# microsoft/aurora

Measured on AMD Instinct MI355X. Metric: forecast-steps/sec (6h step) 0.25deg ERA5 721x1440x13, higher is better.
Workload: dtype bf16; 1 GPU; AuroraPretrained(autocast=True) 1.3B, 0.25deg ERA5 721x1440, 13 levels, T=2, batch 1 per GPU, one forward step (BASELINE.json configs[1]); parallelism=1 GPU

## Files before the change

aurora_amd/csrc/model.h:

```cpp
#pragma once

#include <math.h>
#include <stdlib.h>
#include <string.h>

#include <algorithm>
#include <array>
#include <exception>
#include <map>
#include <memory>
#include <stdexcept>
#include <string>
#include <vector>

#include "band.h"
#include "common.h"

namespace aurora {

struct Fail {
  int code;
};
#define REQUIRE(cond, ...)               \
  do {                                   \
// ... 73 lines not shown
struct Resampler {
  struct Layer {
    const float *to_q, *to_kv, *to_out, *fc1_w, *fc1_b, *fc2_w, *fc2_b, *ln1_w, *ln1_b, *ln2_w, *ln2_b;
    const float *ln_k_w = nullptr, *ln_k_b = nullptr, *ln_q_w = nullptr, *ln_q_b = nullptr;
    int inner, head_dim, hidden, dim, ctx_dim;
    float v_l1;
    int f16_mode;
    const void *to_kv_s = nullptr, *to_out_s = nullptr, *fc1_s = nullptr, *fc2_s = nullptr;
  };
  std::vector<Layer> layers;
  std::vector<DevBuf> own;
  DevBuf vs_w, vs_ws;
  int n_s = 0, n_vs = 0, vs_lq = 0;
};

enum SrcKind { SRC_SURF, SRC_STATIC, SRC_DYN, SRC_ATMOS };
struct Channel {
  std::string name;
  SrcKind kind;
  int src;
  int transform;
  float tw0 = 0.f, tw1 = 0.f, tb = 0.f;
};
struct EmbedPack {
  DevBuf w, ws;
  int K = 0, Kpad = 0, groups = 1;
  float l1 = 0.f;
  std::vector<int> channels;
};
struct HeadGroup {
  std::vector<std::string> names;
  DevBuf w, b;
  int groups = 1;
  DevBuf ws, bs;
  int n_pad = 0;
};

struct DevTables { DevBuf tok, grp; int n_windows = 0, n_tok = 0; bool has_grp = false; };
struct DevPlan {
  DevBuf tok, grp, send_idx;
  int n_windows = 0, n_tok = 0, n_own = 0, n_halo = 0, n_interior = 0;
  int recv_off[2] = {0, 0}, recv_cnt[2] = {0, 0}, send_cnt[2] = {0, 0};
  bool has_grp = false;
};

}

struct aurora_hip_model {
  int D = 0, P = 0, Cl = 0, perceiver_heads = 0, n_stages = 0;
  int enc_depths[4] = {0}, dec_depths[4] = {0}, enc_heads[4] = {0}, dec_heads[4] = {0}, window[3] = {0};
  int enc_depth = 1, dec_depth = 1, max_history = 2, lora_steps = 40, lora_mode = 0;
// ... 35 lines not shown
  std::vector<double> static_loc;
  std::map<std::array<int64_t, 3>, aurora::EmbedPack> embed_packs;
  float enc_bias_max = 0.f;
  aurora::DevBuf surf_w0_s, surf_w2_s;
  float surf_l1_0 = 0.f, surf_b0 = 0.f, surf_c = 0.f;
  bool surf_chain = false;
  aurora::HeadGroup head_surf, head_main, head_alt;
  float dec_out_bound = 0.f, dec_out_bound_alt = 0.f;
  std::map<std::pair<int, int>, aurora::DevTables> tables;
  std::vector<aurora::Res> stage_res;
  std::vector<std::array<int, 2>> merge_pad;

  aurora_hip_band band{0, 1, nullptr, nullptr, nullptr};
  std::vector<std::vector<std::array<int, 2>>> rows;
  std::map<std::pair<int, int>, aurora::DevPlan> plans;
  void* stage_send = nullptr;
  void* stage_recv = nullptr;
  int64_t staging_bytes = 0, staging_need = 0;
  bool sharded() const { return band.world > 1; }
  int fuse_ln = 1;
  bool split_attention = false;
  bool qkv_planes = true;
  bool reassoc_out = true;
  bool score_weights = true;

  aurora::DevBuf abs_enc, dyn_planes, ctx_max;
  aurora::DevBuf tickets;
  bool split_k = true;
  int abs_B = 0;
  struct Pinned { float* host = nullptr; size_t bytes = 0; hipEvent_t done = nullptr; };
  Pinned pinned[4];
  int pinned_next = 0;
  ~aurora_hip_model() {
    for (auto& t : timed) { (void)hipEventDestroy(t.e0); (void)hipEventDestroy(t.e1); }
    for (auto& e : event_pool) (void)hipEventDestroy(e);
    for (auto& s : pinned) {
      if (s.host) (void)hipHostFree(s.host);
      if (s.done) (void)hipEventDestroy(s.done);
    }
  }
  aurora::Arena arena;
  bool dry = false;
  int64_t generation = 0;

  struct Timed { int kind; double work; hipEvent_t e0, e1; };
  uint32_t profile_mask = 0;
// ... 121 lines not shown
  std::vector<float> h(n);
  hip_ok(hipMemcpy(h.data(), dev, n * 4, hipMemcpyDeviceToHost), "download");
  return h;
}
inline std::vector<float> to_host(const Tensor& t) { return to_host(t.f(), (size_t)t.numel); }
inline bool contains(const std::vector<std::string>& v, const std::string& s) { return std::find(v.begin(), v.end(), s) != v.end(); }

constexpr float F16_SAFE = 16384.0f;
constexpr float PRESPLIT_W_MAX = 1000.0f;
int bounded_mode();
std::string level_to_str(double level);

int lora_key(const Model& m, int step);
float absmax(const float* dev, size_t n);
float absmax(const std::vector<float>& h);
inline float absmax(const Tensor& t) { return absmax(t.f(), (size_t)t.numel); }
float max_row_l1(const std::vector<float>& h, int64_t rows, int64_t K, float floor);
bool presplit_shape(int64_t rows, int64_t K, int row_multiple);
DevBuf presplit(const float* w, int64_t rows, int64_t K, int64_t ld, int row_multiple, int groups = 1);
void score_weights(Model& m, Resampler& r, const float* q0, int Lq, int heads);
void build_atmos_heads(Model& m, bool per_level);
const AttnSet& attn_weights(Model& m, int key, void* stream);
const EmbedPack& embed_pack(Model& m, int kind, int T, const std::vector<char>& present);
enum Expansion { POS, SCALE, LEAD_TIME, LEVELS, ABS_TIME };
void fourier(Expansion kind, const double* x, int64_t n, int d, float* out);
const DevTables& tables_for(Model& m, int stage, bool shifted);
const DevPlan& plan_for(Model& m, int stage, bool shifted);
struct StepIO {
  const aurora_hip_step_io* io;
  int B, T;
};
void run_step(Model& m, const StepIO& s, void* stream);

}
```

aurora_amd/csrc/model.hip:

```cpp
#include "model.h"

namespace aurora {

hipEvent_t take_event(Model& m) {
  if (!m.event_pool.empty()) {
    hipEvent_t e = m.event_pool.back();
    m.event_pool.pop_back();
    return e;
  }
  hipEvent_t e;
  hip_ok(hipEventCreate(&e), "hipEventCreate");
  return e;
}

int bounded_mode() {
  static const int mode = getenv("AURORA_F32_GEMM") ? -1 : 2;
  return mode;
}

std::string level_to_str(double level) {
  const double value = round(level * 1000.0) / 1000.0;
  char buf[64];
  if (value == (double)(long long)value) snprintf(buf, sizeof buf, "%lld", (long long)value);
  else {
// ... 153 lines not shown
    names(c->density_channel_surf_vars, c->n_density, m->density_vars);
    names(c->angle_surf_vars, c->n_angle, m->angle_vars);
    if (m->surf_inputs.empty()) m->surf_inputs = m->surf_vars;
    REQUIRE(m->variant == 2 || m->surf_inputs == m->surf_vars, "create: surf_inputs are for the ocean-wave variant");
    if (c->difference_history)
      for (int i = 0; i < c->n_modulation_heads; ++i)
        if (c->difference_history[i] >= 0) m->diff_index[m->mod_heads[i]] = c->difference_history[i];
    REQUIRE(m->static_vars.size() <= 60 && m->surf_inputs.size() <= 60 && m->atmos_vars.size() <= 60, "create: too many variables");
    build_blocks(*m);
    build_channels(*m);
    m->ctx_max = DevBuf(16);
    const auto& tu = c->tuning;
    REQUIRE(tu.fuse_ln >= 0 && tu.fuse_ln <= 3, "create: tuning.fuse_ln = %d (0 default, 1 never, 2 by the fill rule, 3 always)", tu.fuse_ln);
    auto sw = [](int32_t v, bool dflt, const char* what) {
      REQUIRE(v >= 0 && v <= 2, "create: tuning.%s = %d (0 default, 1 off, 2 on)", what, v);
      return v == 0 ? dflt : v == 2;
    };
    m->fuse_ln = tu.fuse_ln == 0 ? 1 : tu.fuse_ln - 1;
    m->split_attention = sw(tu.band_split_attention, false, "band_split_attention");
    m->qkv_planes = sw(tu.qkv_planes, true, "qkv_planes");
    m->split_k = sw(tu.split_k, true, "split_k");
    m->reassoc_out = sw(tu.perceiver_reassoc, true, "perceiver_reassoc");
    m->score_weights = sw(tu.score_weights, true, "score_weights");
    m->tickets = DevBuf(SPLIT_TICKETS * sizeof(int32_t));
    hip_ok(hipMemset(m->tickets.p, 0, SPLIT_TICKETS * sizeof(int32_t)), "hipMemset");
    *out = m.release();
  })
}

extern "C" void aurora_hip_destroy(aurora_hip_model* m) { delete m; }

extern "C" int aurora_hip_set_band(aurora_hip_model* mp, const aurora_hip_band* band) {
  GUARDED({
    REQUIRE(mp != nullptr, "set_band: null model");
    Model& m = *mp;
    if (band == nullptr || band->world <= 1) {
      m.band = aurora_hip_band{0, 1, nullptr, nullptr, nullptr};
    } else {
      REQUIRE(band->rank >= 0 && band->rank < band->world, "set_band: rank %d of %d", band->rank, band->world);
      REQUIRE(band->post && band->wait, "set_band: the halo transport callbacks are required");
      m.band = *band;
    }
    m.have_grid = false;
    m.plans.clear(); m.rows.clear();
    m.stage_send = m.stage_recv = nullptr;
    m.staging_bytes = m.staging_need = 0;
// ... 150 lines not shown
```

aurora_amd/csrc/model_weights.hip:

```cpp
#include "model.h"

namespace aurora {

constexpr int LORA_RANK = 8;

float absmax(const std::vector<float>& h) {
  float mx = 0.f;
  for (float v : h) mx = std::max(mx, fabsf(v));
  return mx;
}
float absmax(const float* dev, size_t n) { return absmax(to_host(dev, n)); }
float max_row_l1(const std::vector<float>& h, int64_t rows, int64_t K, float floor) {
  float best = floor;
  for (int64_t r = 0; r < rows; ++r) {
    float sum = 0.f;
    for (int64_t k = 0; k < K; ++k) sum += fabsf(h[(size_t)r * K + k]);
    best = std::max(best, sum);
  }
  return best;
}

bool presplit_shape(int64_t rows, int64_t K, int row_multiple) { return rows % row_multiple == 0 && K % 32 == 0 && K >= 96; }
DevBuf presplit(const float* w, int64_t rows, int64_t K, int64_t ld, int row_multiple, int groups) {
  if (!presplit_shape(rows, K, row_multiple)) return DevBuf();
// ... 173 lines not shown
        hip_ok(hipStreamSynchronize(as_stream(stream)), "sync");
        src = merged.f();
      }
      const void* use = src;
      if (m.autocast) {
        DevBuf h((size_t)out_f * in_f * 2);
        ok(aurora_hip_convert(src, h.p, out_f * in_f, AURORA_F32, stream));
        hip_ok(hipStreamSynchronize(as_stream(stream)), "sync");
        use = h.p;
        set.own.push_back(std::move(h));
      } else if (key >= 0) {
        set.own.push_back(std::move(merged));
      }
      (which == 0 ? set.qkv : set.proj).push_back(use);
    }
  }
  while (m.attn_sets.size() > 3) {
    bool erased = false;
    for (auto jt = m.attn_sets.begin(); jt != m.attn_sets.end(); ++jt)
      if (jt->first != -1) { m.attn_sets.erase(jt); erased = true; break; }
    if (!erased) break;
  }
  return m.attn_sets.emplace(key, std::move(set)).first->second;
}

const EmbedPack& embed_pack(Model& m, int kind, int T, const std::vector<char>& present) {
  const std::vector<Channel>& chans = kind == 0 ? m.surf_channels : m.atmos_channels;
  int64_t mask = 0, mask_hi = 0;
  REQUIRE(chans.size() <= 126, "more than 126 input channels");
  for (size_t i = 0; i < chans.size(); ++i)
    if (present[i]) (i < 63 ? mask : mask_hi) |= (int64_t)1 << (i % 63);
  const std::array<int64_t, 3> key{(int64_t)kind * 1024 + T, mask, mask_hi};
  auto it = m.embed_packs.find(key);
  if (it != m.embed_packs.end()) return it->second;
  EmbedPack pk;
  for (size_t i = 0; i < chans.size(); ++i)
    if (present[i]) pk.channels.push_back((int)i);
  REQUIRE(!pk.channels.empty(), "no %s variable given", kind == 0 ? "surface-level" : "atmospheric");
  const bool per_level = kind == 1 && !m.level_condition.empty();
  pk.groups = per_level ? m.n_levels : 1;
  const int V = (int)pk.channels.size(), PP = m.P * m.P;
  pk.K = V * T * PP;
  pk.Kpad = round_up(pk.K, 32);
  std::vector<float> host((size_t)pk.groups * m.D * pk.Kpad, 0.f);
  for (int g = 0; g < pk.groups; ++g) {
    const std::string prefix = kind == 0 ? "encoder.surf_token_embeds.weights."
                               : per_level ? "encoder.atmos_token_embeds.layers." + level_to_str(m.levels[g]) + ".weights."
                                           : "encoder.atmos_token_embeds.weights.";
    for (int v = 0; v < V; ++v) {
      const Tensor& t = m.T_(prefix + chans[pk.channels[v]].name);
      REQUIRE(t.shape.size() == 5 && t.shape[0] == m.D && t.shape[2] >= T && t.shape[3] == m.P, "bad patch-embed weight shape");
      const int64_t Tmax = t.shape[2];
      const std::vector<float> wv = to_host(t);
      for (int d = 0; d < m.D; ++d)
        for (int tt = 0; tt < T; ++tt)
          memcpy(&host[((size_t)g * m.D + d) * pk.Kpad + ((size_t)v * T + tt) * PP], &wv[((size_t)d * Tmax + tt) * PP], PP * sizeof(float));
    }
  }
  pk.l1 = max_row_l1(host, (int64_t)pk.groups * m.D, pk.Kpad, 1e-6f);
  pk.w = to_device(host);
  if (bounded_mode() == 2 && absmax(host) < PRESPLIT_W_MAX)
    pk.ws = presplit(pk.w.f(), m.D, pk.Kpad, pk.Kpad, 256, pk.groups);
  return m.embed_packs.emplace(key, std::move(pk)).first->second;
}

void build_atmos_heads(Model& m, bool per_level) {
  std::vector<std::string> sep = m.sep_perceiver, main_names, alt_names;
  if (!m.mod_heads.empty())
    for (const auto& v : m.sep_perceiver) sep.push_back(v + "_mod");
  for (const auto& n : m.atmos_heads) (contains(sep, n) ? alt_names : main_names).push_back(n);
  build_heads(m, m.head_main, "atmos", main_names, per_level);
  build_heads(m, m.head_alt, "atmos", alt_names, per_level);
}

namespace {

void surface_mlp_chain(Model& m) {
  const Tensor &t0 = m.T_("encoder.surf_mlp.net.0.weight"), &t2 = m.T_("encoder.surf_mlp.net.2.weight");
  const std::vector<float> w0 = to_host(t0), w2 = to_host(t2);
  const int64_t N0 = t0.shape[0], K0 = t0.shape[1];
  m.surf_l1_0 = max_row_l1(w0, N0, K0, 1e-6f);
  m.surf_b0 = absmax(m.T_("encoder.surf_mlp.net.0.bias"));
  m.surf_c = absmax(m.T_("encoder.surf_token_embeds.bias")) + absmax(m.T_("encoder.surf_level_encoding"));
  m.surf_chain = bounded_mode() == 2 && absmax(w0) < PRESPLIT_W_MAX && absmax(w2) < PRESPLIT_W_MAX &&
                 presplit_shape(N0, K0, 256) && presplit_shape(K0, N0, 256);
// ... 62 lines not shown
                1e-5f, AURORA_F32);
  hip_ok(hipStreamSynchronize(as_stream(L.stream)), "precompute sync");
  score_weights(m, m.enc_rs, m.enc_q0.f(), n_lat, m.perceiver_heads);
  m.has_alt = !m.sep_perceiver.empty();
  if (m.has_alt) m.dec_rs_alt = pack_resampler(m, "decoder.level_decoder_alternate", m.dec_depth, m.perceiver_heads);
}

void feature_combiners(Model& m) {
  for (int kind = 0; kind < 2; ++kind)
    for (Channel& ch : kind == 0 ? m.surf_channels : m.atmos_channels)
      if (ch.transform == 2) {
        const std::string p = std::string(kind == 0 ? "surf" : "atmos") + "_feature_combiner." + ch.name;
        const std::vector<float> wv = to_host(m.T_(p + ".weight")), bv = to_host(m.T_(p + ".bias"));
        REQUIRE(wv.size() == 2 && bv.size() == 1, "bad feature combiner shape for %s", p.c_str());
        ch.tw0 = wv[0]; ch.tw1 = wv[1]; ch.tb = bv[0];
      }
}

}

}

using namespace aurora;

extern "C" int aurora_hip_pack_weights(aurora_hip_model* m, const char* name, const void* data, const int64_t* shape, int ndim,
                                       int dtype, int on_device) {
  GUARDED({
    REQUIRE(m && name && data && ndim >= 0 && ndim <= 8, "pack_weights: bad argument");
    REQUIRE(dtype == AURORA_F32, "pack_weights: parameters must be float32 (the engine keeps fp32 masters)");
    Tensor t;
    t.numel = 1;
    for (int i = 0; i < ndim; ++i) { t.shape.push_back(shape[i]); t.numel *= shape[i]; }
    t.buf = DevBuf((size_t)t.numel * 4);
    hip_ok(hipMemcpy(t.buf.p, data, (size_t)t.numel * 4, on_device ? hipMemcpyDeviceToDevice : hipMemcpyHostToDevice),
           "pack_weights copy");
    m->w[name] = std::move(t);
    m->finalized = false;
  })
}

namespace {
const char PACK_MAGIC[] = "AURORAHIP1";

bool backbone_matrix(const Model& m, const std::string& name) {
  if (name.rfind("backbone.", 0) != 0 || name.size() < 7 || name.compare(name.size() - 7, 7, ".weight") != 0) return false;
  for (const char* tag : {".mlp.fc1.", ".mlp.fc2.", ".downsample.reduction.", ".upsample.lin1.", ".upsample.lin2."})
// ... 103 lines not shown
```

aurora_amd/csrc/step.hip:

```cpp
#include <algorithm>

#include "model.h"
#include "resampler_space.h"

namespace aurora {

namespace {

struct CtxGuard { const float* word; float a, c, limit_kv; bool pairs; };

LayerSpace layer_space(const Model& m, const Resampler& rs, size_t i, int B, int64_t cols, int64_t ctx_rows, int Lq, int Lk,
                       int heads) {
  const auto& ly = rs.layers[i];
  LayerShape sh{};
  sh.layer = i;
  sh.dim = ly.dim; sh.inner = ly.inner; sh.hidden = ly.hidden; sh.head_dim = ly.head_dim; sh.heads = heads;
  sh.n_vs = rs.n_vs; sh.vs_lq = rs.vs_lq;
  sh.ln_k = ly.ln_k_w != nullptr; sh.to_out_s = ly.to_out_s != nullptr; sh.fc1_s = ly.fc1_s != nullptr; sh.fc2_s = ly.fc2_s != nullptr;
  sh.f16_mode = ly.f16_mode;
  sh.reassoc_out = m.reassoc_out;
  sh.out_supported = aurora_hip_perceiver_out_supported(Lq, Lk, heads, ly.head_dim, ly.dim) != 0;
  sh.B = B; sh.cols = cols; sh.ctx_rows = ctx_rows; sh.Lq = Lq; sh.Lk = Lk;
  return layer_space(sh);
}

void resampler_mlp(Model& m, Launcher& L, const Resampler::Layer& ly, const LayerSpace& sp, const float* o, const float* res,
                   int64_t res_mod, float* lat1, char* S, float* y, int64_t n_rows, float eps, bool y_pairs) {
  const int Dd = ly.dim;
  if (sp.pairs)
    timed(m, L.stream, K_LAYERNORM, 0.0, [&] {
      return aurora_hip_layernorm_split(o, Dd, ly.ln1_w, ly.ln1_b, res, Dd, res_mod, 0, nullptr, 0, lat1, Dd, n_rows, Dd, eps, L.stream);
    });
  else L.layernorm(o, Dd, ly.ln1_w, ly.ln1_b, res, Dd, res_mod, lat1, Dd, nullptr, 0, n_rows, Dd, eps, AURORA_F32);
  float* hid = (float*)S;
  const int64_t chunk_rows = sp.chunk_rows;
  REQUIRE(chunk_rows >= 1 && (size_t)chunk_rows * sp.hid_row <= sp.s_bytes, "resampler: scratch region too small for the MLP");
  const int all = 2 | AURORA_F32_A_SPLIT | AURORA_F32_W_SPLIT;
  for (int64_t r0 = 0; r0 < n_rows; r0 += chunk_rows) {
    const int64_t nr = std::min(chunk_rows, n_rows - r0);
    LinearOp fc1(lat1 + (size_t)r0 * Dd, Dd, sp.pairs ? ly.fc1_s : ly.fc1_w, Dd, ly.fc1_b, hid, ly.hidden, nr, ly.hidden, Dd, AURORA_F32);
    LinearOp fc2(hid, ly.hidden, sp.pairs ? ly.fc2_s : ly.fc2_w, ly.hidden, ly.fc2_b, y + (size_t)r0 * Dd, Dd, nr, Dd, ly.hidden, AURORA_F32);
    L.linear(fc1.activation(AURORA_ACT_GELU).f32_mode(sp.pairs ? all | AURORA_F32_C_SPLIT : ly.f16_mode));
    L.linear(fc2.f32_mode(sp.pairs ? all : ly.f16_mode));
  }
  if (sp.pairs)
    timed(m, L.stream, K_LAYERNORM, 0.0, [&] {
      return aurora_hip_layernorm_split(y, Dd, ly.ln2_w, ly.ln2_b, lat1, Dd, 0, 1, y_pairs ? nullptr : y, Dd, y_pairs ? y : nullptr, Dd,
                                        n_rows, Dd, eps, L.stream);
    });
  else L.layernorm(y, Dd, ly.ln2_w, ly.ln2_b, lat1, Dd, 0, y, Dd, nullptr, 0, n_rows, Dd, eps, AURORA_F32);
}

float* resampler(Model& m, Launcher& L, const Resampler& rs, const float* ctx, int64_t ctx_rows, int ctx_dim, const float* q0,
                 const float* latents0, int B, int64_t cols, int64_t kv_bstride, int64_t kv_lstride, int Lq, int Lk, int heads,
                 float eps, const CtxGuard* cg = nullptr, bool out_pairs = false, int own_word = 0, bool scan_ctx = true) {
  const int64_t n_cols = (int64_t)B * cols, n_rows = n_cols * Lq;
  const float* ctx_max = cg ? cg->word : m.ctx_max.f() + own_word;
  const float g_a = cg ? cg->a : 1.0f, g_c = cg ? cg->c : 0.0f;
  const bool ctx_pairs = cg && cg->pairs;
  if (!cg && scan_ctx)
    timed(m, L.stream, K_ABSMAX, 0.0, [&] { return aurora_hip_absmax_fold(ctx, ctx_rows * ctx_dim, m.ctx_max.f() + own_word, L.stream); });
  float* lat = nullptr;
  for (size_t i = 0; i < rs.layers.size(); ++i) {
    const auto& ly = rs.layers[i];
    const int inner = ly.inner, Dd = ly.dim;
    const LayerSpace sp = layer_space(m, rs, i, B, cols, ctx_rows, Lq, Lk, heads);
    const bool scores = sp.scores;
    const int kv_ld = sp.kv_ld;
    float* y = (float*)m.arena.take(sp.unit);
    const size_t after_y = m.arena.top;
    float* lat1 = (float*)m.arena.take(sp.unit);
    char* S = (char*)m.arena.take(sp.s_bytes);
    float* kv = (float*)S;
    auto guarded = [&](const float* A, int64_t lda, const float* Wf, const void* Ws, float* C_, int64_t ldc, int64_t M_, int N_,
                       int K_, float limit, bool a_pairs = false) {
      LinearOp op(A, lda, Wf, K_, nullptr, C_, ldc, M_, N_, K_, AURORA_F32);
      if (Ws) {
        L.guarded_pair(op, Ws, a_pairs ? AURORA_F32_A_SPLIT : 0, ctx_max, limit);
      } else if (ly.f16_mode == 2) {
        L.linear(op.f32_mode(2).guarded_by(ctx_max, limit));
      } else {
        L.linear(op.f32_mode(ly.f16_mode));
      }
    };
    REQUIRE(!ctx_pairs || ly.to_kv_s, "resampler: a pair-layout context needs pre-split to_kv weights");
    guarded(ctx, ctx_dim, scores ? rs.vs_w.f() : ly.to_kv, scores ? rs.vs_ws.p : ly.to_kv_s, kv, kv_ld, ctx_rows, kv_ld, ctx_dim,
            ctx_pairs ? cg->limit_kv : (F16_SAFE - g_c) / g_a, ctx_pairs);
    if (ly.ln_k_w)
      L.layernorm(kv, 2 * inner, ly.ln_k_w, ly.ln_k_b, nullptr, 0, 0, kv, 2 * inner, nullptr, 0, ctx_rows, inner, 1e-5f,
                  AURORA_F32);
    const float* q = q0;
    int64_t q_stride = 0;
    if (i > 0) {
      float* qb = (float*)(S + round256(sp.kv_bytes));
      L.linear(LinearOp(lat, Dd, ly.to_q, Dd, nullptr, qb, inner, n_rows, inner, Dd, AURORA_F32));
      if (ly.ln_q_w) L.layernorm(qb, inner, ly.ln_q_w, ly.ln_q_b, nullptr, 0, 0, qb, inner, nullptr, 0, n_rows, inner, 1e-5f, AURORA_F32);
      q = qb;
      q_stride = Lq;
    }
    float* att = sp.att_in_y ? y : (float*)(S + sp.att_off);
    const float lim_out = (F16_SAFE / ly.v_l1 - g_c) / g_a;
    float* o = (float*)S;
    if (sp.reassoc) {
      REQUIRE(sp.p_off >= sp.kv_bytes && sp.p_off >= sp.unit && sp.p_off + sp.p_bytes <= sp.s_bytes,
              "resampler: the softmax weights overlap k | v or to_out's result in the scratch region");
      float* P = (float*)(S + sp.p_off);
      void* Vp = y;
      timed(m, L.stream, K_PERCEIVER_ATTENTION, 0.0, [&] {
        if (scores)
          return aurora_hip_perceiver_probs_scores(kv, kv_ld, inner, P, Vp, B, cols, kv_bstride, kv_lstride, Lq, Lk, heads, ly.head_dim,
                                                   ctx_max, lim_out, L.stream);
        return aurora_hip_perceiver_probs(q, kv, P, Vp, B, cols, kv_bstride, kv_lstride, Lq, Lk, heads, ly.head_dim, ctx_max, lim_out,
                                          L.stream);
      });
      timed(m, L.stream, K_PERCEIVER_OUT, 2.0 * (double)n_cols * Lk * Dd * inner + 2.0 * (double)n_rows * Dd * heads * Lk, [&] {
        return aurora_hip_perceiver_out(Vp, ly.to_out_s, inner, P, nullptr, o, Dd, n_cols, Lq, Lk, heads, ly.head_dim, Dd, ctx_max,
                                        lim_out, L.stream);
      });
      timed(m, L.stream, K_PERCEIVER_ATTENTION, 0.0, [&] {
        if (scores)
          return aurora_hip_perceiver_attention_scores(kv, kv_ld, inner, att, B, cols, kv_bstride, kv_lstride, Lq, Lk, heads,
                                                       ly.head_dim, nullptr, 0.f, ctx_max, lim_out, L.stream);
        return aurora_hip_perceiver_attention_unless(q, q_stride, kv, att, B, cols, kv_bstride, kv_lstride, Lq, Lk, heads,
                                                     ly.head_dim, AURORA_F32, nullptr, 0.f, ctx_max, lim_out, L.stream);
// ... 130 lines not shown
    const float lim_e = F16_SAFE, lim_0 = (F16_SAFE - m.surf_c) / l1e, lim_2 = ((F16_SAFE - m.surf_b0) / m.surf_l1_0 - m.surf_c) / l1e;
    L.guarded_pair(embed, ps.ws.p, 0, word, lim_e);
    L.guarded_pair(fc1, m.surf_w0_s.p, 0, word, lim_0);
    L.guarded_pair(fc2, m.surf_w2_s.p, 0, word, lim_2);
  } else {
    L.linear(embed);
    L.linear(fc1);
    L.linear(fc2);
  }
  L.layernorm(y, D, m.W("encoder.surf_norm.weight"), m.W("encoder.surf_norm.bias"), xs0, D, 0, y, D, nullptr, 0, R, D, 1e-5f,
              AURORA_F32);
  return y;
}

const float* encode_levels(Step& s) {
  Model& m = s.m;
  Launcher& L = s.L;
  const int B = s.B, D = s.D, C = s.C;
  float* A_a;
  const EmbedPack& pa = embed_input(s, true, A_a);
  const int Kpad_a = pa.Kpad;
  bool chain = pa.ws.p != nullptr;
  for (const auto& ly : m.enc_rs.layers) chain = chain && ly.f16_mode == 2 && ly.to_kv_s != nullptr;
  float* word = m.ctx_max.f() + 1;
  patchify(s, pa, true, A_a, chain ? word : nullptr);
  float* xa = (float*)m.arena.take((size_t)C * B * s.Lp * D * 4);
  const int64_t R = (int64_t)B * s.Lp;
  CtxGuard cg{};
  const int64_t sw = pa.groups > 1 ? (int64_t)D * Kpad_a : 0;
  const LinearOp embed = LinearOp(A_a, Kpad_a, pa.w.f(), Kpad_a, m.enc_bias.f(), xa, D, R, D, Kpad_a, AURORA_F32)
                             .batched(C, R * Kpad_a, sw, D, R * D);
  if (chain) {
    const float l1 = pa.l1, cb = m.enc_bias_max;
    cg = CtxGuard{word, l1, cb, std::min(F16_SAFE, (F16_SAFE - cb) / l1), true};
    L.guarded_pair(embed, pa.ws.p, AURORA_F32_C_SPLIT, cg.word, cg.limit_kv);
  } else {
    L.linear(embed);
  }
  return resampler(m, L, m.enc_rs, xa, (int64_t)C * R, D, m.enc_q0.f(), m.W("encoder.atmos_latents"), B, s.Lp, s.Lp, R, s.Cl - 1, C,
                   m.perceiver_heads, m.ln_eps, chain ? &cg : nullptr);
}

void assemble(Step& s, const float* xs1, const float* lat, float* x_f, void* x_b) {
  Model& m = s.m;
  const int B = s.B, D = s.D;
  float* time_emb = (float*)m.arena.take((size_t)B * D * 4);
  s.L.linear(LinearOp(m.abs_enc.f(), D, m.W("encoder.absolute_time_embed.weight"), D, m.W("encoder.absolute_time_embed.bias"), time_emb,
                      D, B, D, D, AURORA_F32).residual(m.lead_emb.f(), 0));
  timed(m, s.L.stream, K_ASSEMBLE, 0.0, [&] {
    return aurora_hip_assemble_tokens(xs1, lat, m.pos_scale.f(), time_emb, x_f, x_b, B, s.Cl, s.Lp, D, s.bb, s.L.stream);
// ... 397 lines not shown
```

aurora_amd/engine/lib.py:

```python

from __future__ import annotations

import ctypes
import os
import threading
from collections import OrderedDict, namedtuple
from ctypes import c_float, c_int, c_int32, c_int64, c_void_p
from pathlib import Path
from typing import Optional

import numpy as np
import torch

F32, BF16, F64 = 0, 1, 2
ACT_NONE, ACT_GELU, ACT_SILU = 0, 1, 2

_LIB_PATH = Path(__file__).resolve().parents[1] / "_lib" / "libaurora_hip.so"


class PatchVar(ctypes.Structure):
    _fields_ = [
        ("src", c_void_p), ("stride_b", c_int64), ("stride_t", c_int64), ("stride_c", c_int64),
        ("stride_h", c_int64), ("stride_w", c_int64), ("loc", c_void_p), ("inv_scale", c_void_p),
        ("transform", c_int32), ("tw0", c_float), ("tw1", c_float), ("tb", c_float),
# ... 1320 lines not shown
    with torch.cuda.device(dev):
        order = [what for what, _ in groups if what in addr]
        table = _plane_table("diagnostics", tuple(a for what in order for a in addr[what]), dev)
        at, first = {}, table.data_ptr()
        for what in order:
            at[what], first = first, first + 8 * len(addr[what])
        moved = 4.0 * n_lat * n_lon * (n_wind * (2 + sum(k in addr for k in ("vo", "div", "ws"))) +
                                       n_cols * (C * (1 + sum(k in addr for k in ("col_u", "col_v"))) +
                                                 sum(k in addr for k in ("tcwv", "ivtu", "ivtv", "ivt"))))
        with _Timed("diagnostics", moved):
            _check(load().aurora_hip_diagnostics(at.get("u"), at.get("v"), at.get("vo"), at.get("div"), at.get("ws"), n_wind,
                                                 _ptr(row_table), float(L), 1 if wrap else 0, at.get("q"), at.get("col_u"),
                                                 at.get("col_v"), at.get("tcwv"), at.get("ivtu"), at.get("ivtv"), at.get("ivt"),
                                                 n_cols, C, _ptr(level_w), n_lat, n_lon, _stream()))


_PD =ctypes.POINTER(ctypes.c_double)
_PF = ctypes.POINTER(ctypes.c_float)
_PS = ctypes.POINTER(ctypes.c_char_p)


class HipTuning(ctypes.Structure):
    _fields_ = [("fuse_ln", c_int32), ("band_split_attention", c_int32), ("qkv_planes", c_int32), ("split_k", c_int32),
                ("perceiver_reassoc", c_int32), ("score_weights", c_int32), ("reserved", c_int32 * 2)]


def tuning_from_env() -> HipTuning:
    t = HipTuning()

    def value(var: str, allowed: tuple[int, ...]):
        raw = os.environ.get(var)
        if raw is None:
            return None
        try:
            v = int(raw.strip())
        except ValueError:
            v = None
        if v not in allowed:
            raise ValueError(f"{var}={raw!r}: expected one of {', '.join(map(str, allowed))}")
        return v

    v = value("AURORA_FUSE_LN", (0, 1, 2))
    if v is not None:
        t.fuse_ln = v + 1
    for field, var in (("band_split_attention", "AURORA_BAND_SPLIT_ATTENTION"), ("qkv_planes", "AURORA_QKV_PLANES"),
                       ("split_k", "AURORA_SPLIT_K"), ("perceiver_reassoc", "AURORA_PERCEIVER_REASSOC"),
                       ("score_weights", "AURORA_SCORE_WEIGHTS")):
        v = value(var, (0, 1))
        if v is not None:
            setattr(t, field, 2 if v else 1)
    return t


class HipConfig(ctypes.Structure):
    _fields_ = [("embed_dim", c_int32), ("patch_size", c_int32), ("latent_levels", c_int32), ("num_heads", c_int32),
                ("n_stages", c_int32), ("encoder_depths", c_int32 * 4), ("encoder_heads", c_int32 * 4),
                ("decoder_depths", c_int32 * 4), ("decoder_heads", c_int32 * 4), ("window", c_int32 * 3),
                ("enc_depth", c_int32), ("dec_depth", c_int32), ("perceiver_ln_eps", c_float),
                ("max_history", c_int32), ("timestep_hours", ctypes.c_double), ("stabilise_level_agg", c_int32),
                ("use_lora", c_int32), ("lora_steps", c_int32), ("lora_mode", c_int32), ("autocast", c_int32),
                ("n_surf", c_int32), ("n_static", c_int32), ("n_atmos", c_int32),
                ("surf_vars", _PS), ("static_vars", _PS), ("atmos_vars", _PS),
                ("variant", c_int32), ("n_level_condition", c_int32), ("level_condition", _PD),
                ("dynamic_vars", c_int32), ("atmos_static_vars", c_int32), ("clamp_at_first_step", c_int32),
                ("simulate_indexing_bug", c_int32),
                ("n_separate_perceiver", c_int32), ("separate_perceiver", _PS),
                ("n_modulation_heads", c_int32), ("modulation_heads", _PS),
                ("difference_history", ctypes.POINTER(c_int32)),
                ("n_positive_surf", c_int32), ("positive_surf_vars", _PS),
                ("n_positive_atmos", c_int32), ("positive_atmos_vars", _PS),
# ... 41 lines not shown


PROFILE_KINDS = ("linear_bf16", "linear_f32", "window_attention_bf16", "layernorm", "merge_ln", "split_ln", "patchify",
                 "perceiver_attention", "assemble_tokens", "unpatchify", "copy2d", "absmax", "linear_layernorm_bf16",
                 "gather_rows", "perceiver_out")

_SIGNATURES.update({
    "aurora_hip_profile_begin": (c_int, [c_void_p, ctypes.c_uint32]),
    "aurora_hip_profile_end": (c_int, [c_void_p, ctypes.POINTER(HipProfileEntry), c_int, ctypes.POINTER(c_int)]),
    "aurora_hip_profile_end_list": (c_int, [c_void_p, ctypes.POINTER(HipProfileEntry), c_int, ctypes.POINTER(c_int)]),
    "aurora_hip_create": (c_int, [ctypes.POINTER(HipConfig), ctypes.POINTER(c_void_p)]),
    "aurora_hip_destroy": (None, [c_void_p]),
    "aurora_hip_pack_weights": (c_int, [c_void_p, ctypes.c_char_p, c_void_p, ctypes.POINTER(c_int64), c_int, c_int, c_int]),
    "aurora_hip_finalize": (c_int, [c_void_p, c_void_p]),
    "aurora_hip_save_packed": (c_int, [c_void_p, ctypes.c_char_p, c_void_p]),
    "aurora_hip_load_packed": (c_int, [c_void_p, ctypes.c_char_p]),
    "aurora_hip_precompute": (c_int, [c_void_p, ctypes.POINTER(HipGrid), c_void_p]),
    "aurora_hip_set_time": (c_int, [c_void_p, _PD, c_int, c_void_p]),
    "aurora_hip_step": (c_int, [c_void_p, ctypes.POINTER(HipStepIO), c_void_p]),
    "aurora_hip_workspace_bytes": (c_int64, [c_void_p]),
    "aurora_hip_guard_words": (c_int, [c_void_p, ctypes.POINTER(c_float), c_void_p]),
    "aurora_hip_abi_sizes": (c_int, [ctypes.POINTER(c_int32), c_int]),
    "aurora_hip_generation": (c_int64, [c_void_p]),
    "aurora_hip_output_vars": (c_int, [c_void_p, _PS, c_int]),
    "aurora_hip_set_time_ex": (c_int, [c_void_p, _PD, ctypes.POINTER(c_int32), c_int, c_void_p]),
    "aurora_hip_set_band": (c_int, [c_void_p, ctypes.POINTER(HipBand)]),
    "aurora_hip_band_rows": (c_int, [c_void_p, ctypes.POINTER(c_int32), ctypes.POINTER(c_int32)]),
    "aurora_hip_band_staging_bytes": (c_int64, [c_void_p]),
    "aurora_hip_set_band_staging": (c_int, [c_void_p, c_void_p, c_void_p, c_int64]),
    "aurora_hip_pos_scale_encoding": (c_int, [_PD, _PD, c_int, c_int, c_int, c_int, _PF, _PF]),
    "aurora_hip_band_partition": (c_int, [c_int, ctypes.POINTER(c_int32), ctypes.POINTER(c_int32), c_int, c_int, c_int,
                                          ctypes.POINTER(c_int32), ctypes.POINTER(c_int32)]),
    "aurora_hip_band_plan": (c_int, [ctypes.POINTER(c_int32), ctypes.POINTER(c_int32), c_int, c_int, c_int,
                                     ctypes.POINTER(c_int32), ctypes.POINTER(HipPlanInfo), c_void_p, c_void_p, c_void_p,
                                     c_void_p]),
})
EXPORTED_SYMBOLS = tuple(_SIGNATURES)
```

aurora_amd/engine/native.py:

```python
from __future__ import annotations

import ctypes
from datetime import timedelta

import numpy as np
import torch

from aurora_amd import normalisation
from aurora_amd.batch import BandBatch, Batch, derive_metadata
from aurora_amd.engine import encodings, lib

_LORA_MODES = {"single": 0, "from_second": 1, "all": 2}
_VARIANTS = {"base": 0, "air_pollution": 1, "wave": 2}


def _version(t: torch.Tensor) -> int:
    try:
        return t._version
    except RuntimeError:
        return -1


def _strs(names):
    return (ctypes.c_char_p * max(len(names), 1))(*[n.encode() for n in names])
# ... 275 lines not shown
        lib._check(lib.load().aurora_hip_profile_end(self._h, out, len(out), ctypes.byref(n)))
        return {e.kernel.decode(): {"launches": e.launches, "ms": e.ms, "work": e.work} for e in out[:n.value] if e.launches}

    def profile_end_list(self) -> list:
        n = ctypes.c_int(0)
        lib._check(lib.load().aurora_hip_profile_end_list(self._h, None, 0, ctypes.byref(n)))
        out = (lib.HipProfileEntry * max(n.value, 1))()
        lib._check(lib.load().aurora_hip_profile_end_list(self._h, out, n.value, ctypes.byref(n)))
        return [(e.kernel.decode(), e.ms, e.work) for e in out[:n.value]]

    def set_time(self, times) -> None:
        stamps = _dbl([t.timestamp() / 3600 for t in times])
        cal = _i32([x for t in times for x in (t.hour, t.weekday(), t.day)])
        lib._check(lib.load().aurora_hip_set_time_ex(self._h, stamps, cal, len(times), lib._stream()))

    def workspace_bytes(self) -> int:
        return int(lib.load().aurora_hip_workspace_bytes(self._h))

    def guard_words(self) -> tuple[float, float, float, float]:
        out = (ctypes.c_float * 4)()
        lib._check(lib.load().aurora_hip_guard_words(self._h, out, lib._stream()))
        return tuple(float(v) for v in out)

    def generation(self) -> int:
        return int(lib.load().aurora_hip_generation(self._h))

    @torch.no_grad()
    def step(self, batch: Batch, upload_time: bool = True, out=None) -> Batch:
        cfg = self.cfg
        md = batch.metadata
        levels = tuple(md.atmos_levels)
        H, W = batch.spatial_shape
        first = next(iter(batch.surf_vars.values()))
        B, T = first.shape[:2]
        dev = first.device
        assert md.lat.shape[0] == H and md.lon.shape[-1] == W
        assert md.lat.dtype in (torch.float32, torch.float64), f"Latitude num. unstable: {md.lat.dtype}."
        assert md.lon.dtype in (torch.float32, torch.float64), f"Longitude num. unstable: {md.lon.dtype}."
        if self.shard is None:
            self.precompute(md.lat, md.lon, levels)
        else:
            assert self.band_rows is not None and H == self.band_rows[1] - self.band_rows[0], "not this rank's latitude band"
        if upload_time:
            self.set_time(md.time)

        def unknown(d_, known, what):
# ... 62 lines not shown
```

include/aurora_hip.h:

```cpp
#ifndef AURORA_HIP_H
#define AURORA_HIP_H

#include <stddef.h>
#include <stdint.h>

#ifdef __cplusplus
extern "C" {
#endif

#define AURORA_F32 0
#define AURORA_BF16 1
#define AURORA_F64 2

#define AURORA_OK 0
#define AURORA_E_ARG (-1)
#define AURORA_E_LAUNCH (-2)

#define AURORA_ACT_NONE 0
#define AURORA_ACT_GELU 1
#define AURORA_ACT_SILU 2

const char* aurora_hip_last_error(void);
int aurora_hip_version(void);

// ... 176 lines not shown
  int32_t n_surf, n_static, n_atmos;
  const char* const* surf_vars;
  const char* const* static_vars;
  const char* const* atmos_vars;
  int32_t variant;
  int32_t n_level_condition;
  const double* level_condition;
  int32_t dynamic_vars, atmos_static_vars, clamp_at_first_step, simulate_indexing_bug;
  int32_t n_separate_perceiver;  const char* const* separate_perceiver;
  int32_t n_modulation_heads;    const char* const* modulation_heads;
  const int32_t* difference_history;
  int32_t n_positive_surf;       const char* const* positive_surf_vars;
  int32_t n_positive_atmos;      const char* const* positive_atmos_vars;
  int32_t n_surf_inputs;         const char* const* surf_inputs;
  int32_t n_density;             const char* const* density_channel_surf_vars;
  int32_t n_angle;               const char* const* angle_surf_vars;
  struct aurora_hip_tuning {
    int32_t fuse_ln;
    int32_t band_split_attention;
    int32_t qkv_planes;
    int32_t split_k;
    int32_t perceiver_reassoc;
    int32_t score_weights;
    int32_t reserved[2];
  } tuning;
} aurora_hip_config;

typedef struct aurora_hip_grid {
  int32_t n_lat, n_lon;
  const double* lat;
  const double* lon;
  int32_t n_levels;
  const double* levels;
  int32_t levels_float32;
  const double* surf_loc;
  const double* surf_scale;
  const double* static_loc;
  const double* static_scale;
  const double* atmos_loc;
  const double* atmos_scale;
  const float* pos_encoding;
  const float* scale_encoding;
} aurora_hip_grid;

typedef struct aurora_hip_step_io {
  int32_t B, T;
  const float* const* surf;
// ... 2 lines not shown
  int64_t static_strides[2];
  const float* const* atmos;
  int64_t atmos_strides[5];
  float* const* out_surf;
  float* const* out_atmos;
  int32_t rollout_step;
} aurora_hip_step_io;

int aurora_hip_create(const aurora_hip_config* config, aurora_hip_model** out);
void aurora_hip_destroy(aurora_hip_model* model);
int aurora_hip_pack_weights(aurora_hip_model* model, const char* name, const void* data, const int64_t* shape, int ndim,
                            int dtype, int on_device);
int aurora_hip_finalize(aurora_hip_model* model, void* stream);
int aurora_hip_save_packed(aurora_hip_model* model, const char* path, void* stream);
int aurora_hip_load_packed(aurora_hip_model* model, const char* path);
int aurora_hip_precompute(aurora_hip_model* model, const aurora_hip_grid* grid, void* stream);
int aurora_hip_pos_scale_encoding(const double* lat, const double* lon, int n_lat, int n_lon, int patch_size,
                                  int embed_dim, float* pos_out, float* scale_out);
int aurora_hip_set_time(aurora_hip_model* model, const double* time_hours, int B, void* stream);
int aurora_hip_step(aurora_hip_model* model, const aurora_hip_step_io* io, void* stream);
int64_t aurora_hip_workspace_bytes(const aurora_hip_model* model);
#define AURORA_F16_SAFE_RANGE 16384.0f
int aurora_hip_guard_words(const aurora_hip_model* model, float out[4], void* stream);
int64_t aurora_hip_generation(const aurora_hip_model* model);
int aurora_hip_abi_sizes(int32_t* out, int capacity);
int aurora_hip_output_vars(const aurora_hip_model* model, const char** names, int capacity);
int aurora_hip_set_time_ex(aurora_hip_model* model, const double* time_hours, const int32_t* calendar, int B, void* stream);

typedef struct aurora_hip_halo_msg {
  int32_t peer;
  int32_t reserved;
  int64_t offset;
  int64_t bytes;
} aurora_hip_halo_msg;
typedef int (*aurora_hip_halo_post_fn)(void* user, const aurora_hip_halo_msg* sends, int32_t n_sends,
                                       const aurora_hip_halo_msg* recvs, int32_t n_recvs, void* stream);
typedef int (*aurora_hip_halo_wait_fn)(void* user, void* stream);
typedef struct aurora_hip_band {
  int32_t rank, world;
  aurora_hip_halo_post_fn post;
  aurora_hip_halo_wait_fn wait;
  void* user;
} aurora_hip_band;
int aurora_hip_set_band(aurora_hip_model* model, const aurora_hip_band* band);
int aurora_hip_band_rows(const aurora_hip_model* model, int32_t* row0, int32_t* row1);
int64_t aurora_hip_band_staging_bytes(const aurora_hip_model* model);
// ... 114 lines not shown
```

Baseline: 7.867 forecast-steps/s.

## Fold encoder patch embedding into perceiver context key/value projections

The atmospheric patch-embedding weights and bias are pre-multiplied into each encoder perceiver layer's to_kv (or score) weights on the host, at pack time. The resampler then projects raw patch pixels straight to keys and values, skipping the intermediate D-dimensional embedding tensor and its GEMM. A FLOP-count rule decides whether the fold is applied, and a new bound on composed weights keeps the half-precision guard limits valid. In exchange, composed weights use extra memory and host compute at pack time, and rounding changes slightly because the product is reassociated.

```diff
diff --git a/aurora_amd/csrc/model.h b/aurora_amd/csrc/model.h
--- a/aurora_amd/csrc/model.h
+++ b/aurora_amd/csrc/model.h
@@ -119,11 +119,17 @@
   int transform;
   float tw0 = 0.f, tw1 = 0.f, tb = 0.f;
 };
+struct ComposedCtx {
+  DevBuf w, ws, bias;
+  int N = 0;
+  float v_l1 = 0.f, vb_max = 0.f;
+};
 struct EmbedPack {
   DevBuf w, ws;
   int K = 0, Kpad = 0, groups = 1;
   float l1 = 0.f;
   std::vector<int> channels;
+  std::vector<ComposedCtx> composed;
 };
 struct HeadGroup {
   std::vector<std::string> names;
@@ -205,6 +211,8 @@
   bool split_attention = false;
   bool qkv_planes = true;
   bool reassoc_out = true;
+  bool compose_front = true;
+  bool front_composed = false;
   bool score_weights = true;
 
   aurora::DevBuf abs_enc, dyn_planes, ctx_max;
@@ -372,6 +380,14 @@
 void build_atmos_heads(Model& m, bool per_level);
 const AttnSet& attn_weights(Model& m, int key, void* stream);
 const EmbedPack& embed_pack(Model& m, int kind, int T, const std::vector<char>& present);
+struct ValueBound {
+  float a, c;
+  float word_limit() const { return (F16_SAFE - c) / a; }
+};
+inline ValueBound composed_value_bound(float v_l1, float embed_l1, float embed_bias_max, float composed_v_l1, float composed_vb_max) {
+  return ValueBound{std::min(composed_v_l1, v_l1 * embed_l1), std::min(composed_vb_max, v_l1 * embed_bias_max)};
+}
+bool compose_front_rule(int Kpad, int D, const int* N, int n_layers);
 enum Expansion { POS, SCALE, LEAD_TIME, LEVELS, ABS_TIME };
 void fourier(Expansion kind, const double* x, int64_t n, int d, float* out);
 const DevTables& tables_for(Model& m, int stage, bool shifted);
diff --git a/aurora_amd/csrc/model.hip b/aurora_amd/csrc/model.hip
--- a/aurora_amd/csrc/model.hip
+++ b/aurora_amd/csrc/model.hip
@@ -199,6 +199,7 @@
     m->split_k = sw(tu.split_k, true, "split_k");
     m->reassoc_out = sw(tu.perceiver_reassoc, true, "perceiver_reassoc");
     m->score_weights = sw(tu.score_weights, true, "score_weights");
+    m->compose_front = sw(tu.compose_front, true, "compose_front");
     m->tickets = DevBuf(SPLIT_TICKETS * sizeof(int32_t));
     hip_ok(hipMemset(m->tickets.p, 0, SPLIT_TICKETS * sizeof(int32_t)), "hipMemset");
     *out = m.release();
diff --git a/aurora_amd/csrc/model_weights.hip b/aurora_amd/csrc/model_weights.hip
--- a/aurora_amd/csrc/model_weights.hip
+++ b/aurora_amd/csrc/model_weights.hip
@@ -219,6 +219,60 @@
     if (!erased) break;
   }
   return m.attn_sets.emplace(key, std::move(set)).first->second;
+}
+
+bool compose_front_rule(int Kpad, int D, const int* N, int n_layers) {
+  if (Kpad <= 0 || D <= 0 || n_layers <= 0) return false;
+  double composed = 0.0, staged = (double)Kpad * D;
+  for (int i = 0; i < n_layers; ++i) {
+    if (N[i] <= 0) return false;
+    composed += (double)Kpad * N[i];
+    staged += (double)D * N[i];
+  }
+  return 2.0 * composed <= staged;
+}
+
+namespace {
+
+void compose_front(Model& m, EmbedPack& pk) {
+  const Resampler& rs = m.enc_rs;
+  if (!m.compose_front || rs.layers.empty() || m.enc_bias.p == nullptr) return;
+  const int D = m.D, C = m.n_levels, Kpad = pk.Kpad;
+  std::vector<int> N;
+  for (size_t i = 0; i < rs.layers.size(); ++i) {
+    if (rs.layers[i].ctx_dim != D) return;
+    N.push_back(i == 0 && rs.n_vs > 0 ? rs.n_vs : 2 * rs.layers[i].inner);
+  }
+  if (!compose_front_rule(Kpad, D, N.data(), (int)N.size())) return;
+  const std::vector<float> we = to_host(pk.w.f(), (size_t)pk.groups * D * Kpad), eb = to_host(m.enc_bias.f(), (size_t)C * D);
+  std::vector<ComposedCtx> out;
+  for (size_t i = 0; i < rs.layers.size(); ++i) {
+    const auto& ly = rs.layers[i];
+    const bool scores = i == 0 && rs.n_vs > 0;
+    const int n = N[i], v0 = scores ? 0 : ly.inner;
+    const std::vector<float> wc = to_host(scores ? rs.vs_w.f() : ly.to_kv, (size_t)n * D);
+    std::vector<float> w((size_t)pk.groups * n * Kpad), b((size_t)C * n);
+    ok(aurora_hip_compose_weight(wc.data(), n, D, we.data(), Kpad, pk.groups, w.data()));
+    ok(aurora_hip_compose_bias(wc.data(), n, D, eb.data(), C, b.data()));
+    if (!(absmax(w) < PRESPLIT_W_MAX)) return;
+    ComposedCtx cc;
+    cc.N = n;
+    cc.v_l1 = 1e-6f;
+    for (int g = 0; g < pk.groups; ++g) {
+      const auto first = w.begin() + ((size_t)g * n + v0) * Kpad;
+      cc.v_l1 = max_row_l1(std::vector<float>(first, first + (size_t)ly.inner * Kpad), ly.inner, Kpad, cc.v_l1);
+    }
+    for (int c = 0; c < C; ++c)
+      for (int r = 0; r < ly.inner; ++r) cc.vb_max = std::max(cc.vb_max, fabsf(b[(size_t)c * n + v0 + r]));
+    cc.w = to_device(w);
+    cc.bias = to_device(b);
+    if (ly.f16_mode == 2 && pk.ws.p != nullptr && (scores ? rs.vs_ws.p : ly.to_kv_s) != nullptr)
+      cc.ws = presplit(cc.w.f(), n, Kpad, Kpad, 256, pk.groups);
+    out.push_back(std::move(cc));
+  }
+  pk.composed = std::move(out);
+}
+
 }
 
 const EmbedPack& embed_pack(Model& m, int kind, int T, const std::vector<char>& present) {
@@ -258,6 +312,7 @@
   pk.w = to_device(host);
   if (bounded_mode() == 2 && absmax(host) < PRESPLIT_W_MAX)
     pk.ws = presplit(pk.w.f(), m.D, pk.Kpad, pk.Kpad, 256, pk.groups);
+  if (kind == 1) compose_front(m, pk);
   return m.embed_packs.emplace(key, std::move(pk)).first->second;
 }
 
@@ -366,6 +421,54 @@
 }
 
 using namespace aurora;
+
+extern "C" int aurora_hip_compose_weight(const float* w_ctx, int N, int D, const float* w_e, int K, int groups, float* out) {
+  GUARDED({
+    REQUIRE(w_ctx && w_e && out && N > 0 && D > 0 && K > 0 && groups > 0, "compose_weight: bad argument");
+    std::vector<double> acc((size_t)K);
+    for (int g = 0; g < groups; ++g)
+      for (int n = 0; n < N; ++n) {
+        std::fill(acc.begin(), acc.end(), 0.0);
+        for (int d = 0; d < D; ++d) {
+          const double a = w_ctx[(size_t)n * D + d];
+          const float* row = w_e + ((size_t)g * D + d) * K;
+          for (int k = 0; k < K; ++k) acc[k] += a * row[k];
+        }
+        float* dst = out + ((size_t)g * N + n) * K;
+        for (int k = 0; k < K; ++k) dst[k] = (float)acc[k];
+      }
+  })
+}
+
+extern "C" int aurora_hip_compose_bias(const float* w_ctx, int N, int D, const float* bias, int C, float* out) {
+  GUARDED({
+    REQUIRE(w_ctx && bias && out && N > 0 && D > 0 && C > 0, "compose_bias: bad argument");
+    for (int c = 0; c < C; ++c)
+      for (int n = 0; n < N; ++n) {
+        double acc = 0.0;
+        for (int d = 0; d < D; ++d) acc += (double)w_ctx[(size_t)n * D + d] * bias[(size_t)c * D + d];
+        out[(size_t)c * N + n] = (float)acc;
+      }
+  })
+}
+
+extern "C" int aurora_hip_compose_front_rule(int Kpad, int D, const int32_t* N, int n_layers) {
+  return compose_front_rule(Kpad, D, N, n_layers) ? 1 : 0;
+}
+
+extern "C" int aurora_hip_composed_value_bound(float v_l1, float embed_l1, float embed_bias_max, float composed_v_l1,
+                                               float composed_vb_max, float out[6]) {
+  GUARDED({
+    REQUIRE(out && v_l1 > 0.f && embed_l1 > 0.f && composed_v_l1 > 0.f && embed_bias_max >= 0.f && composed_vb_max >= 0.f,
+            "composed_value_bound: bad argument");
+    const ValueBound staged{v_l1 * embed_l1, v_l1 * embed_bias_max}, folded = composed_value_bound(v_l1, embed_l1, embed_bias_max,
+                                                                                              composed_v_l1, composed_vb_max);
+    out[0] = staged.a; out[1] = staged.c; out[2] = (F16_SAFE / v_l1 - embed_bias_max) / embed_l1;
+    out[3] = folded.a; out[4] = folded.c; out[5] = folded.word_limit();
+  })
+}
+
+extern "C" int aurora_hip_front_composed(const aurora_hip_model* m) { return m != nullptr && m->front_composed ? 1 : 0; }
 
 extern "C" int aurora_hip_pack_weights(aurora_hip_model* m, const char* name, const void* data, const int64_t* shape, int ndim,
                                        int dtype, int on_device) {
diff --git a/aurora_amd/csrc/step.hip b/aurora_amd/csrc/step.hip
--- a/aurora_amd/csrc/step.hip
+++ b/aurora_amd/csrc/step.hip
@@ -8,6 +8,7 @@
 namespace {
 
 struct CtxGuard { const float* word; float a, c, limit_kv; bool pairs; };
+struct ComposedFront { const ComposedCtx* layers; int levels, groups; int64_t rows; float embed_l1, embed_bias_max; };
 
 LayerSpace layer_space(const Model& m, const Resampler& rs, size_t i, int B, int64_t cols, int64_t ctx_rows, int Lq, int Lk,
                        int heads) {
@@ -53,7 +54,8 @@
 
 float* resampler(Model& m, Launcher& L, const Resampler& rs, const float* ctx, int64_t ctx_rows, int ctx_dim, const float* q0,
                  const float* latents0, int B, int64_t cols, int64_t kv_bstride, int64_t kv_lstride, int Lq, int Lk, int heads,
-                 float eps, const CtxGuard* cg = nullptr, bool out_pairs = false, int own_word = 0, bool scan_ctx = true) {
+                 float eps, const CtxGuard* cg = nullptr, bool out_pairs = false, int own_word = 0, bool scan_ctx = true,
+                 const ComposedFront* front = nullptr) {
   const int64_t n_cols = (int64_t)B * cols, n_rows = n_cols * Lq;
   const float* ctx_max = cg ? cg->word : m.ctx_max.f() + own_word;
   const float g_a = cg ? cg->a : 1.0f, g_c = cg ? cg->c : 0.0f;
@@ -84,8 +86,19 @@
       }
     };
     REQUIRE(!ctx_pairs || ly.to_kv_s, "resampler: a pair-layout context needs pre-split to_kv weights");
-    guarded(ctx, ctx_dim, scores ? rs.vs_w.f() : ly.to_kv, scores ? rs.vs_ws.p : ly.to_kv_s, kv, kv_ld, ctx_rows, kv_ld, ctx_dim,
-            ctx_pairs ? cg->limit_kv : (F16_SAFE - g_c) / g_a, ctx_pairs);
+    if (front) {
+      const ComposedCtx& cc = front->layers[i];
+      REQUIRE(cc.N == kv_ld && front->levels * front->rows == ctx_rows, "resampler: composed context weights of another shape");
+      LinearOp op = LinearOp(ctx, ctx_dim, cc.w.f(), ctx_dim, cc.bias.f(), kv, kv_ld, front->rows, kv_ld, ctx_dim, AURORA_F32)
+                        .batched(front->levels, front->rows * ctx_dim, front->groups > 1 ? (int64_t)kv_ld * ctx_dim : 0, kv_ld,
+                                 front->rows * kv_ld);
+      if (cc.ws.p) L.guarded_pair(op, cc.ws.p, 0, ctx_max, F16_SAFE);
+      else if (ly.f16_mode == 2) L.linear(op.f32_mode(2).guarded_by(ctx_max, F16_SAFE));
+      else L.linear(op.f32_mode(ly.f16_mode));
+    } else {
+      guarded(ctx, ctx_dim, scores ? rs.vs_w.f() : ly.to_kv, scores ? rs.vs_ws.p : ly.to_kv_s, kv, kv_ld, ctx_rows, kv_ld, ctx_dim,
+              ctx_pairs ? cg->limit_kv : (F16_SAFE - g_c) / g_a, ctx_pairs);
+    }
     if (ly.ln_k_w)
       L.layernorm(kv, 2 * inner, ly.ln_k_w, ly.ln_k_b, nullptr, 0, 0, kv, 2 * inner, nullptr, 0, ctx_rows, inner, 1e-5f,
                   AURORA_F32);
@@ -99,7 +112,9 @@
       q_stride = Lq;
     }
     float* att = sp.att_in_y ? y : (float*)(S + sp.att_off);
-    const float lim_out = (F16_SAFE / ly.v_l1 - g_c) / g_a;
+    const float lim_out = front ? composed_value_bound(ly.v_l1, front->embed_l1, front->embed_bias_max, front->layers[i].v_l1,
+                                                       front->layers[i].vb_max).word_limit()
+                                : (F16_SAFE / ly.v_l1 - g_c) / g_a;
     float* o = (float*)S;
     if (sp.reassoc) {
       REQUIRE(sp.p_off >= sp.kv_bytes && sp.p_off >= sp.unit && sp.p_off + sp.p_bytes <= sp.s_bytes,
@@ -276,10 +291,20 @@
   const int Kpad_a = pa.Kpad;
   bool chain = pa.ws.p != nullptr;
   for (const auto& ly : m.enc_rs.layers) chain = chain && ly.f16_mode == 2 && ly.to_kv_s != nullptr;
+  const bool composed = !pa.composed.empty();
+  m.front_composed = composed;
   float* word = m.ctx_max.f() + 1;
-  patchify(s, pa, true, A_a, chain ? word : nullptr);
+  patchify(s, pa, true, A_a, chain || composed ? word : nullptr);
+  const int64_t R = (int64_t)B * s.Lp;
+  if (composed) {
+    REQUIRE(pa.composed.size() == m.enc_rs.layers.size(), "encoder: composed context weights for %zu of %zu layers",
+            pa.composed.size(), m.enc_rs.layers.size());
+    const CtxGuard cgc{word, 1.0f, 0.0f, F16_SAFE, false};
+    const ComposedFront front{pa.composed.data(), C, pa.groups, R, pa.l1, m.enc_bias_max};
+    return resampler(m, L, m.enc_rs, A_a, (int64_t)C * R, Kpad_a, m.enc_q0.f(), m.W("encoder.atmos_latents"), B, s.Lp, s.Lp, R,
+                     s.Cl - 1, C, m.perceiver_heads, m.ln_eps, &cgc, false, 0, true, &front);
+  }
   float* xa = (float*)m.arena.take((size_t)C * B * s.Lp * D * 4);
-  const int64_t R = (int64_t)B * s.Lp;
   CtxGuard cg{};
   const int64_t sw = pa.groups > 1 ? (int64_t)D * Kpad_a : 0;
   const LinearOp embed = LinearOp(A_a, Kpad_a, pa.w.f(), Kpad_a, m.enc_bias.f(), xa, D, R, D, Kpad_a, AURORA_F32)
diff --git a/aurora_amd/engine/lib.py b/aurora_amd/engine/lib.py
--- a/aurora_amd/engine/lib.py
+++ b/aurora_amd/engine/lib.py
@@ -1366,7 +1366,8 @@
 
 class HipTuning(ctypes.Structure):
     _fields_ = [("fuse_ln", c_int32), ("band_split_attention", c_int32), ("qkv_planes", c_int32), ("split_k", c_int32),
-                ("perceiver_reassoc", c_int32), ("score_weights", c_int32), ("reserved", c_int32 * 2)]
+                ("perceiver_reassoc", c_int32), ("score_weights", c_int32), ("compose_front", c_int32),
+                ("reserved", c_int32 * 1)]
 
 
 def tuning_from_env() -> HipTuning:
@@ -1389,7 +1390,7 @@
         t.fuse_ln = v + 1
     for field, var in (("band_split_attention", "AURORA_BAND_SPLIT_ATTENTION"), ("qkv_planes", "AURORA_QKV_PLANES"),
                        ("split_k", "AURORA_SPLIT_K"), ("perceiver_reassoc", "AURORA_PERCEIVER_REASSOC"),
-                       ("score_weights", "AURORA_SCORE_WEIGHTS")):
+                       ("score_weights", "AURORA_SCORE_WEIGHTS"), ("compose_front", "AURORA_COMPOSE_FRONT")):
         v = value(var, (0, 1))
         if v is not None:
             setattr(t, field, 2 if v else 1)
@@ -1477,6 +1478,11 @@
     "aurora_hip_guard_words": (c_int, [c_void_p, ctypes.POINTER(c_float), c_void_p]),
     "aurora_hip_abi_sizes": (c_int, [ctypes.POINTER(c_int32), c_int]),
     "aurora_hip_generation": (c_int64, [c_void_p]),
+    "aurora_hip_compose_weight": (c_int, [_PF, c_int, c_int, _PF, c_int, c_int, _PF]),
+    "aurora_hip_compose_bias": (c_int, [_PF, c_int, c_int, _PF, c_int, _PF]),
+    "aurora_hip_compose_front_rule": (c_int, [c_int, c_int, ctypes.POINTER(c_int32), c_int]),
+    "aurora_hip_composed_value_bound": (c_int, [c_float, c_float, c_float, c_float, c_float, _PF]),
+    "aurora_hip_front_composed": (c_int, [c_void_p]),
     "aurora_hip_output_vars": (c_int, [c_void_p, _PS, c_int]),
     "aurora_hip_set_time_ex": (c_int, [c_void_p, _PD, ctypes.POINTER(c_int32), c_int, c_void_p]),
     "aurora_hip_set_band": (c_int, [c_void_p, ctypes.POINTER(HipBand)]),
diff --git a/aurora_amd/engine/native.py b/aurora_amd/engine/native.py
--- a/aurora_amd/engine/native.py
+++ b/aurora_amd/engine/native.py
@@ -321,6 +321,9 @@
         lib._check(lib.load().aurora_hip_guard_words(self._h, out, lib._stream()))
         return tuple(float(v) for v in out)
 
+    def front_composed(self) -> bool:
+        return bool(lib.load().aurora_hip_front_composed(self._h))
+
     def generation(self) -> int:
         return int(lib.load().aurora_hip_generation(self._h))
 
diff --git a/include/aurora_hip.h b/include/aurora_hip.h
--- a/include/aurora_hip.h
+++ b/include/aurora_hip.h
@@ -222,7 +222,8 @@
     int32_t split_k;
     int32_t perceiver_reassoc;
     int32_t score_weights;
-    int32_t reserved[2];
+    int32_t compose_front;
+    int32_t reserved[1];
   } tuning;
 } aurora_hip_config;
 
@@ -271,6 +272,12 @@
 int64_t aurora_hip_workspace_bytes(const aurora_hip_model* model);
 #define AURORA_F16_SAFE_RANGE 16384.0f
 int aurora_hip_guard_words(const aurora_hip_model* model, float out[4], void* stream);
+int aurora_hip_compose_weight(const float* w_ctx, int N, int D, const float* w_e, int K, int groups, float* out);
+int aurora_hip_compose_bias(const float* w_ctx, int N, int D, const float* bias, int C, float* out);
+int aurora_hip_compose_front_rule(int Kpad, int D, const int32_t* N, int n_layers);
+int aurora_hip_composed_value_bound(float v_l1, float embed_l1, float embed_bias_max, float composed_v_l1,
+                                    float composed_vb_max, float out[6]);
+int aurora_hip_front_composed(const aurora_hip_model* model);
 int64_t aurora_hip_generation(const aurora_hip_model* model);
 int aurora_hip_abi_sizes(int32_t* out, int capacity);
 int aurora_hip_output_vars(const aurora_hip_model* model, const char** names, int capacity);
```

Result: faster. 7.967 forecast-steps/s (median of 6 runs) (+1.3%).
